# dspcraft/dsc

Measured on AMD Instinct MI355X. Metric: batched 1-D rfft GSamples/s, higher is better.
Workload: dtype f32

## Files before the change

### dsc_amd/csrc/check_store_hazard.py

```python
#!/usr/bin/env python3
import os
import re
import struct
import subprocess
import sys
import tempfile

LLVM = '/opt/rocm/lib/llvm/bin'
BUNDLE_MAGIC = b'__CLANG_OFFLOAD_BUNDLE__'

_STORE = re.compile(r'^(buffer|global|flat|scratch)_store_(dwordx3|dwordx4|b96|b128)\s+(.*)$')
_VREG = re.compile(r'v\[(\d+):(\d+)\]|v(\d+)\b')
_NOP = re.compile(r'^s_nop\s+(\d+)')


def _vrange(tok):
    m = _VREG.match(tok.strip())
    if not m:
        return None
    if m.group(3) is not None:
        return int(m.group(3)), int(m.group(3))
    return int(m.group(1)), int(m.group(2))


def _valu_dest(instr):
    if not instr.startswith('v_'):
        return None
    op, _, rest = instr.partition(' ')
    if op.startswith(('v_cmp', 'v_cmpx', 'v_readlane', 'v_readfirstlane', 'v_nop')):
        return None
    first = rest.split(',')[0]
    return _vrange(first)


def device_code_objects(path):
    data = open(path, 'rb').read()
    found = False
    pos = 0
    while True:
        i = data.find(BUNDLE_MAGIC, pos)
        if i < 0:
            break
        n = struct.unpack_from('<Q', data, i + 24)[0]
        off = i + 32
        for _ in range(n):
            o, size, tsz = struct.unpack_from('<QQQ', data, off)
            off += 24
            triple = data[off:off + tsz].decode()
            off += tsz
            if 'amdgcn' in triple and size:
                found = True
                yield f'{os.path.basename(path)}@{i + o}', data[i + o:i + o + size]
        pos = i + 24
    if not found and data[:4] == b'\x7fELF' and data[18:20] == b'\xe0\x00':
        yield os.path.basename(path), data


def disassemble(blob):
    with tempfile.NamedTemporaryFile(suffix='.co') as f:
        f.write(blob)
        f.flush()
        out = subprocess.run([f'{LLVM}/llvm-objdump', '-d', '--no-show-raw-insn', '--no-leading-addr', f.name], check=True, capture_output=True, text=True).stdout
    return out


def scan_text(asm, label=''):
    stores = 0
    bad = []
    func = '?'
    lines = []
    for raw in asm.splitlines():
        s = raw.split('//')[0].split(';')[0].strip()
        if not s:
            continue
        if s.endswith(':') and not s.startswith(('v_', 's_', 'buffer_', 'global_', 'ds_', 'flat_', 'scratch_')):
            func = s.rstrip(':').strip('<>')
            m = re.match(r'^[0-9a-f]+ <(.*)>$', func)
            if m:
                func = m.group(1)
            lines.append(('label', func))
            continue
        lines.append(('i', s))
    cur = '?'
    for idx, (kind, s) in enumerate(lines):
        if kind == 'label':
            if not s.startswith(('.L', 'L')):
                cur = s
            continue
        m = _STORE.match(s)
        if not m:
            continue
        ops = [o.strip() for o in m.group(3).split(',')]
        data = _vrange(ops[0] if m.group(1) == 'buffer' else (ops[1] if len(ops) > 1 else ''))
        if data is None:
            continue
        stores += 1
        need = 2 if m.group(1) == 'buffer' else 1
        ws = 0
        k = idx + 1
        while ws < need and k < len(lines):
            kind2, t = lines[k]
            k += 1
            if kind2 == 'label':
                continue
            d = _valu_dest(t)
            if d is not None and d[0] <= data[1] and d[1] >= data[0]:
                bad.append(f'{label} {cur}: `{s}` then, {ws} wait state(s) later, `{t}`')
                break
            nop = _NOP.match(t)
            ws += int(nop.group(1)) + 1 if nop else 1
            if t.startswith(('s_endpgm', 's_branch', 's_setpc')):
                break
    return stores, bad


def scan_file(path):
    total, bad = 0, []
    for label, blob in device_code_objects(path):
        n, b = scan_text(disassemble(blob), label)
        total += n
        bad += b
    return total, bad


def main(argv):
    total, bad = 0, []
    for p in argv:
        n, b = scan_file(p)
        total += n
        bad += b
    print(f'check_store_hazard: {total} stores of more than 64 bits, {len(bad)} with a VALU write to their data registers inside the wait states')
    for line in bad[:40]:
        print('  ' + line)
    return 1 if bad or total == 0 else 0


if __name__ == '__main__':
    sys.exit(main(sys.argv[1:]))
```

### dsc_amd/csrc/fft_c2c_32k.hip

```cpp
#define DSC_R2C64K_HELPERS_ONLY 1
#include "fft_r2c_64k.hip"

namespace {

template<bool INV, bool CAST>
__global__ __launch_bounds__(1024) void c2c32k_kernel(const f2 *__restrict__ z, f2 *__restrict__ Z, int batch, const f2 *__restrict__ aux,
                                                      int in_pitch, int in_len) {
    constexpr int EB = CAST ? 4 : 8;
    auto sample = [](__amdgpu_buffer_rsrc_t r, int voff, int soff) {
        if constexpr (CAST) return cf{__builtin_bit_cast(float, __builtin_amdgcn_raw_buffer_load_b32(r, voff, soff, kStream)), 0.0f};
        else return load_c(r, voff, soff);
    };
    extern __shared__ __attribute__((aligned(16))) float lds[];
    float *plane = lds;
    f2 *T = (f2 *) (lds + kPlaneFloats);
    fill_twiddle_table(T, aux);
    const int wave_sgpr = __builtin_amdgcn_readfirstlane(threadIdx.x >> 6);
    constexpr float kScale = 1.0f / (float) kM;

    cf v[32];
    {
        const int row0 = blockIdx.x;
        const __amdgpu_buffer_rsrc_t r0 = __builtin_amdgcn_make_buffer_rsrc(
            (void *) ((const char *) z + (size_t) row0 * in_pitch * EB), 0, row0 < batch ? in_len * EB : 0, 0x00020000);
        const int load_off = thread_id(wave_sgpr) * EB;
#pragma unroll
        for (int a = 0; a < 32; ++a) v[a] = sample(r0, load_off, a * 1024 * EB);
    }
    for (int row = blockIdx.x; row < batch; row += gridDim.x) {
        const int next_row = row + gridDim.x;
        const __amdgpu_buffer_rsrc_t rnext = __builtin_amdgcn_make_buffer_rsrc(
            (void *) ((const char *) z + (size_t) next_row * in_pitch * EB), 0, next_row < batch ? in_len * EB : 0, 0x00020000);
        const __amdgpu_buffer_rsrc_t rout = __builtin_amdgcn_make_buffer_rsrc((void *) (Z + (size_t) row * kM), 0, kM * 8, 0x00020000);
        three_passes<INV>(v, plane, T, aux, wave_sgpr, wave_sgpr, false, false);
        if (INV) {
#pragma unroll
            for (int p = 0; p < 32; ++p) v[p] = cf{v[p].x * kScale, v[p].y * kScale};
        }
        const int load_off = thread_id(wave_sgpr) * EB;
        staged_time_store(v, plane, rout, wave_sgpr, [&](bool first_half) {
            if (first_half) {
#pragma unroll
                for (int a = 0; a < 16; ++a) v[2 * a] = sample(rnext, load_off, a * 1024 * EB);
            } else {
#pragma unroll
                for (int a = 16; a < 32; ++a) v[2 * (a - 16) + 1] = sample(rnext, load_off, a * 1024 * EB);
            }
        });
        unzip_rows(v);
    }
}

}

void dsc_launch_fft32k_c32(const void *z, void *Z, int batch, int in_pitch, int in_len, bool inverse, bool cast, const void *aux, int n_cu,
                           hipStream_t stream) {
    if (batch <= 0) return;
    const int grid = batch < n_cu ? batch : n_cu;
    with_bool(inverse, [&](auto inv) { with_bool(cast, [&](auto c) {
        dsc_launch_dyn_lds<c2c32k_kernel<decltype(inv)::value, decltype(c)::value>>(grid, 1024, kLdsBytes, stream, (const f2 *) z, (f2 *) Z, batch,
                                                                                    (const f2 *) aux, in_pitch, in_len);
    }); });
}
```

### dsc_amd/csrc/fft_r2c_64k.hip

```cpp
#include "dispatch.h"

#include <hip/hip_runtime.h>

#include <cmath>
#include <cstdlib>
#include <utility>

namespace {

typedef float f2 __attribute__((ext_vector_type(2)));

struct cf { float x, y; };
__device__ __forceinline__ cf operator+(cf a, cf b) { return cf{a.x + b.x, a.y + b.y}; }
__device__ __forceinline__ cf operator-(cf a, cf b) { return cf{a.x - b.x, a.y - b.y}; }
__device__ __forceinline__ cf to_cf(f2 a) { return cf{a.x, a.y}; }
__device__ __forceinline__ f2 to_f2(cf a) { return f2{a.x, a.y}; }

constexpr int kM = 32768;
constexpr int kPlaneFloats = 1024 * 34;
constexpr int kLdsBytes = kPlaneFloats * 4 + 1024 * 8;
constexpr int kTabEntries = 1024;

constexpr int kAuxW1024 = 0, kAuxW32768 = 1024, kAuxW65536 = 2048, kAuxEntries = 3072;

__host__ __device__ constexpr int br5(int x) {
    return ((x & 1) << 4) | ((x & 2) << 2) | (x & 4) | ((x & 8) >> 2) | ((x & 16) >> 4);
}

__device__ constexpr float kCos64[17] = {
    1.0f, 0.99518472667219688624f, 0.98078528040323044913f, 0.95694033573220886494f,
    0.92387953251128675613f, 0.88192126434835502971f, 0.83146961230254523708f, 0.77301045336273696081f,
    0.70710678118654752440f, 0.63439328416364549822f, 0.55557023301960222474f, 0.47139673682599764856f,
    0.38268343236508977173f, 0.29028467725446236764f, 0.19509032201612826785f, 0.09801714032956060199f,
    0.0f};

__device__ constexpr float root64_re(int q) {
    q &= 63;
    return q <= 16 ? kCos64[q] : q <= 32 ? -kCos64[32 - q] : q <= 48 ? -kCos64[q - 32] : kCos64[64 - q];
}
__device__ constexpr float root64_im(int q) {
    q &= 63;
    return q <= 16 ? -kCos64[16 - q] : q <= 32 ? -kCos64[q - 16] : q <= 48 ? kCos64[48 - q] : kCos64[q - 48];
}

__device__ __forceinline__ cf cmul(cf a, cf w) {
    return cf{a.x * w.x - a.y * w.y, a.x * w.y + a.y * w.x};
}
__device__ __forceinline__ cf cmul_conj(cf a, cf w) {
    return cf{a.x * w.x + a.y * w.y, a.y * w.x - a.x * w.y};
}

template<bool INV>
__device__ __forceinline__ cf twiddle_mul_second_fused(cf a, cf w) {
    if (INV) return cf{__builtin_fmaf(a.y, w.y, a.x * w.x), __builtin_fmaf(-a.x, w.y, a.y * w.x)};
    return cf{__builtin_fmaf(-a.y, w.y, a.x * w.x), __builtin_fmaf(a.y, w.x, a.x * w.y)};
}

template<bool INV, int M, int K>
__device__ __forceinline__ cf mul_root(cf d) {
    constexpr float c8 = 0.70710678118654752440f;
    if constexpr (K == 0) {
        return d;
    } else if constexpr (4 * K == M) {
        return INV ? cf{-d.y, d.x} : cf{d.y, -d.x};
    } else if constexpr (8 * K == M) {
        return INV ? cf{(d.x - d.y) * c8, (d.x + d.y) * c8} : cf{(d.x + d.y) * c8, (d.y - d.x) * c8};
    } else if constexpr (8 * K == 3 * M) {
        return INV ? cf{-(d.x + d.y) * c8, (d.x - d.y) * c8} : cf{(d.y - d.x) * c8, -(d.x + d.y) * c8};
    } else {
        constexpr float wr = root64_re(K * (64 / M));
        constexpr float wi = INV ? -root64_im(K * (64 / M)) : root64_im(K * (64 / M));
        return cf{d.x * wr - d.y * wi, d.x * wi + d.y * wr};
    }
}
// ... 118 lines not shown
#endif

typedef unsigned int u2 __attribute__((ext_vector_type(2)));
typedef unsigned int u4 __attribute__((ext_vector_type(4)));
typedef float f4 __attribute__((ext_vector_type(4)));

#ifndef DSC_LDS_SPLIT_READS
#define DSC_LDS_SPLIT_READS 1
#endif
__device__ __forceinline__ f2 lds_read_b64(const f2 *p) {
#if DSC_LDS_SPLIT_READS
    return *(const volatile __attribute__((address_space(3))) f2 *) p;
#else
    return *p;
#endif
}

__device__ __forceinline__ void lds_barrier() {
    __builtin_amdgcn_fence(__ATOMIC_RELEASE, "workgroup", "local");
    __builtin_amdgcn_s_barrier();
    __builtin_amdgcn_fence(__ATOMIC_ACQUIRE, "workgroup", "local");
}

__device__ __forceinline__ float bperm(int byte_addr, float x) {
    return __int_as_float(__builtin_amdgcn_ds_bpermute(byte_addr, __float_as_int(x)));
}

__device__ __forceinline__ int column_of(int wave, int lane) {
    int kp = lane < 32 ? 32 * wave + lane : 1024 - 32 * wave - (63 - lane);
    return kp == 1024 ? 512 : kp;
}

#ifdef DSC_R2C64K_PROBE
#define PROBE_ARGS , int io_on
#define PROBE_NULL , 1
#define IO_ON io_on
#else
#define PROBE_ARGS
#define PROBE_NULL
#define IO_ON 1
#endif

__device__ __forceinline__ int thread_id(int wave_sgpr) {
    int zero;
    asm volatile("v_mov_b32 %0, 0" : "=v"(zero));
    const int lane = __builtin_amdgcn_mbcnt_hi(-1, __builtin_amdgcn_mbcnt_lo(-1, zero));
    return (wave_sgpr << 6) | lane;
}

#ifndef DSC_STREAM_AUX
#define DSC_STREAM_AUX 2
#endif
constexpr int kStream = DSC_STREAM_AUX;
__device__ __forceinline__ cf load_c(__amdgpu_buffer_rsrc_t r, int voff, int soff) {
    return to_cf(__builtin_bit_cast(f2, __builtin_amdgcn_raw_buffer_load_b64(r, voff, soff, kStream)));
}
#ifndef DSC_FILTER_EARLY_LOADS
#define DSC_FILTER_EARLY_LOADS 4
#endif
#ifndef DSC_IRFFT_PIN_PASS3
#define DSC_IRFFT_PIN_PASS3 1
#endif
#ifndef DSC_IRFFT_EARLY_PAIRS
#define DSC_IRFFT_EARLY_PAIRS 4
#endif
#ifndef DSC_IRFFT_LOAD_AUX
#define DSC_IRFFT_LOAD_AUX 0
#endif
__device__ __forceinline__ cf load_c_spec(__amdgpu_buffer_rsrc_t r, int voff, int soff) {
    return to_cf(__builtin_bit_cast(f2, __builtin_amdgcn_raw_buffer_load_b64(r, voff, soff, DSC_IRFFT_LOAD_AUX)));
}
__device__ __forceinline__ cf load_c_cached(__amdgpu_buffer_rsrc_t r, int voff, int soff) {
    return to_cf(__builtin_bit_cast(f2, __builtin_amdgcn_raw_buffer_load_b64(r, voff, soff, 0)));
}
template<int POLICY>
__device__ __forceinline__ void store_c(cf a, __amdgpu_buffer_rsrc_t r, int voff, int soff) {
    __builtin_amdgcn_raw_buffer_store_b64(__builtin_bit_cast(u2, to_f2(a)), r, voff, soff, POLICY);
}

__device__ __forceinline__ void fill_twiddle_table(f2 *T, const f2 *aux) {
    const int t = threadIdx.x;
    T[t] = aux[kAuxW1024 + (t >> 5) * (t & 31)];
    __syncthreads();
}

constexpr int kCPitch = 33;
static_assert(512 * kCPitch * 8 <= kPlaneFloats * 4, "the step buffer lives inside the plane");

__host__ __device__ constexpr int class_of(int k) { return (k ^ (k >> 1)) & 1; }
__host__ __device__ constexpr int index_in_class(int k) { return ((k >> 2) << 1) | (k & 1); }
static_assert(class_of(br5(0)) == 0 && class_of(br5(7)) == 0 && class_of(br5(24)) == 0 && class_of(br5(31)) == 0 &&
              class_of(br5(8)) == 1 && class_of(br5(23)) == 1, "class 0 = quarters 0 and 3 of a dft32 output");

__device__ __forceinline__ int reader_column(int t) {
    const int a = t >> 5;
    return (t & 31) | ((((a >> 3) | ((a & 7) << 2))) << 5);
}
__device__ __forceinline__ int spectrum_wave(int wave_sgpr) { return (wave_sgpr >> 2) | ((wave_sgpr & 3) << 2); }

template<int Q>
__device__ __forceinline__ void quarter_write(f2 *buf, int wbase, const cf (&v)[32]) {
    int wbase_hi = wbase + 8 * (32 * kCPitch);
    asm("" : "+v"(wbase_hi));
    f2 *lo8 = buf + wbase;
    f2 *hi8 = buf + wbase_hi;
#pragma unroll
    for (int p = 8 * Q; p < 8 * Q + 8; ++p)
        if (index_in_class(br5(p)) < 8) lo8[index_in_class(br5(p)) * (32 * kCPitch)] = to_f2(v[p]);
#pragma unroll
    for (int p = 8 * Q; p < 8 * Q + 8; ++p)
        if (index_in_class(br5(p)) >= 8) hi8[(index_in_class(br5(p)) - 8) * (32 * kCPitch)] = to_f2(v[p]);
}

__device__ __forceinline__ void step_read(const f2 *buf, int row, cf (&dst)[32]) {
    const f2 *r = buf + __mul24(row, kCPitch);
#pragma unroll
    for (int m = 0; m < 32; ++m) dst[m] = to_cf(lds_read_b64(r + m));
}

__device__ __forceinline__ void pin(cf (&v)[32]) {
#pragma unroll
    for (int p = 0; p < 32; p += 8)
        asm volatile("" : "+v"(v[p].x), "+v"(v[p].y), "+v"(v[p + 1].x), "+v"(v[p + 1].y), "+v"(v[p + 2].x), "+v"(v[p + 2].y), "+v"(v[p + 3].x),
                     "+v"(v[p + 3].y), "+v"(v[p + 4].x), "+v"(v[p + 4].y), "+v"(v[p + 5].x), "+v"(v[p + 5].y), "+v"(v[p + 6].x), "+v"(v[p + 6].y),
                     "+v"(v[p + 7].x), "+v"(v[p + 7].y));
}

template<typename Finish>
__device__ __forceinline__ void exchange(f2 *buf, int wbase, int rclass, int rrow, cf (&src)[32], cf (&dst)[32], Finish finish) {
    pin(src);
    lds_barrier();
    finish(std::integral_constant<int, 0>{});
    quarter_write<0>(buf, wbase, src);
    finish(std::integral_constant<int, 3>{});
    quarter_write<3>(buf, wbase, src);
    lds_barrier();
    cf r[32];
    if (rclass == 0) step_read(buf, rrow, r);
    finish(std::integral_constant<int, 1>{});
    lds_barrier();
    quarter_write<1>(buf, wbase, src);
    finish(std::integral_constant<int, 2>{});
    quarter_write<2>(buf, wbase, src);
    lds_barrier();
    if (rclass != 0) step_read(buf, rrow, r);
#pragma unroll
    for (int m = 0; m < 32; ++m) dst[m] = r[m];
}

struct no_hook { __device__ __forceinline__ void operator()() const {} };

template<bool INV, typename Hook = no_hook>
__device__ __forceinline__ void three_passes(cf (&v)[32], float *plane, const f2 *T, const f2 *aux, int wave_sgpr, int col_wave,
                                             bool mirrored_in, bool mirrored_out, Hook before_pass3 = Hook{}) {
    f2 *buf = (f2 *) plane;
    const int wave_class = ((wave_sgpr >> 2) ^ (wave_sgpr >> 3)) & 1;
    dft32_head<INV>(v);
    cf u[32];
    {
        const int t = thread_id(wave_sgpr);
        const int col = mirrored_in ? column_of(col_wave, t & 63) : t;
        const int hi = col >> 5;
        const f2 *th = T + hi;
        const int rc = reader_column(t);
        exchange(buf, __mul24(col & 31, kCPitch) + hi, wave_class, (index_in_class(rc >> 5) << 5) | (rc & 31), v, u, [&](auto Q) {
            constexpr int kQ = decltype(Q)::value;
            dft32_quarter<INV, kQ>(v);
#pragma unroll
            for (int p = 8 * kQ; p < 8 * kQ + 8; ++p) {
                if (p == 0) continue;
                const cf w = to_cf(th[32 * br5(p)]);
                v[p] = INV ? cmul_conj(v[p], w) : cmul(v[p], w);
            }
        });
    }
    dft32_head<INV>(u);
    {
        const int t = thread_id(wave_sgpr);
        const int rc = reader_column(t);
        const int hi = rc >> 5, lo = rc & 31;
        const cf tw2_base = to_cf(aux[kAuxW32768 + __mul24(hi, lo)]);
        const f2 *tl = T + lo;
        const int col_out = mirrored_out ? column_of(col_wave, t & 63) : rc;
        const int k2 = col_out >> 5;
        const int rclass = mirrored_out ? class_of(k2) : wave_class;
        exchange(buf, __mul24(hi, kCPitch) + lo, rclass, (index_in_class(k2) << 5) | (col_out & 31), u, v, [&](auto Q) {
            constexpr int kQ = decltype(Q)::value;
            dft32_quarter<INV, kQ>(u);
#ifdef DSC_DFT32_DIF
            constexpr bool kSumsOnly = false;
#else
            constexpr bool kSumsOnly = true;
#endif
#pragma unroll
            for (int p = 8 * kQ; p < 8 * kQ + 8; ++p) {
                const cf w = p == 0 ? tw2_base : cmul(tw2_base, to_cf(tl[32 * br5(p)]));
                if (kSumsOnly && p < 4) u[p] = twiddle_mul_second_fused<INV>(u[p], w);
                else u[p] = INV ? cmul_conj(u[p], w) : cmul(u[p], w);
            }
        });
    }
    before_pass3();
    dft32<INV>(v);
}

__device__ __forceinline__ void real_pair(cf p, cf q, cf wq, float hs, cf &out_k, cf &out_mk) {
    const cf s = cf{p.x + q.x, p.y - q.y};
    const cf d = cf{p.x - q.x, p.y + q.y};
    const cf wd = cmul(d, wq);
    out_k = cf{hs * s.x + wd.x, hs * s.y + wd.y};
    out_mk = cf{hs * s.x - wd.x, wd.y - hs * s.y};
}

__device__ __forceinline__ int partner_byte_addr(int wave, int lane) {
    return ((wave == 0 && (lane == 63 || lane == 0)) ? lane : 63 - lane) * 4;
}

#ifndef DSC_R2C64K_HELPERS_ONLY
__global__ __launch_bounds__(1024) void rfft64k_kernel(const float *__restrict__ x, f2 *__restrict__ X, int batch,
                                                       const f2 *__restrict__ aux, int in_pitch, int in_len PROBE_ARGS) {
    extern __shared__ __attribute__((aligned(16))) float lds[];
    float *plane = lds;
    f2 *T = (f2 *) (lds + kPlaneFloats);
    fill_twiddle_table(T, aux);

    const int wave_sgpr = __builtin_amdgcn_readfirstlane(threadIdx.x >> 6);

    cf v[32];
    {
        const int row0 = blockIdx.x;
        const __amdgpu_buffer_rsrc_t r0 = __builtin_amdgcn_make_buffer_rsrc(
            (void *) (x + (size_t) row0 * in_pitch), 0, row0 < batch ? in_len * 4 * IO_ON : 0, 0x00020000);
        const int load_off = thread_id(wave_sgpr) * 8;
#pragma unroll
        for (int j1 = 0; j1 < 32; ++j1) v[j1] = load_c(r0, load_off, j1 * 8192);
    }

    for (int row = blockIdx.x; row < batch; row += gridDim.x) {
        const int next_row = row + gridDim.x;
        const __amdgpu_buffer_rsrc_t rnext = __builtin_amdgcn_make_buffer_rsrc(
            (void *) (x + (size_t) next_row * in_pitch), 0, next_row < batch ? in_len * 4 * IO_ON : 0, 0x00020000);
        const __amdgpu_buffer_rsrc_t rout =
            __builtin_amdgcn_make_buffer_rsrc((void *) (X + (size_t) row * (kM + 1)), 0, (kM + 1) * 8 * IO_ON, 0x00020000);

        const int cw = spectrum_wave(wave_sgpr);
        three_passes<false>(v, plane, T, aux, wave_sgpr, cw, false, true);

        const int t4 = thread_id(wave_sgpr);
        const int lane = t4 & 63, wave = t4 >> 6;
        const int kp = column_of(cw, lane);
        const int partner_addr = partner_byte_addr(cw, lane);
        cf xk[16], xm[16];
        const cf zmid = v[br5(16)];
        if (cw == 0) {
#pragma unroll
            for (int r = 16; r < 31; ++r) v[br5(r)] = lane == 0 ? v[br5(r + 1)] : v[br5(r)];
            v[br5(31)] = lane == 0 ? v[br5(0)] : v[br5(31)];
        }
#pragma unroll
        for (int k3 = 0; k3 < 16; ++k3) {
            const int src = 31 - br5(k3);
            xm[k3].x = bperm(partner_addr, v[src].x);
            xm[k3].y = bperm(partner_addr, v[src].y);
        }
        {
            const cf wpost = to_cf(aux[kAuxW65536 + kp]);
            const cf post_base = cf{0.5f * wpost.y, -0.5f * wpost.x};
#pragma unroll
            for (int k3 = 0; k3 < 16; ++k3) {
                const cf c = cf{root64_re(k3), root64_im(k3)};
                const cf w = k3 == 0 ? post_base : cmul(post_base, c);
                real_pair(v[br5(k3)], xm[k3], w, 0.5f, xk[k3], xm[k3]);
            }
        }

        f2 *stage = (f2 *) plane;
        const int skew = (int) ((((size_t) (X + (size_t) row * (kM + 1))) >> 3) & 15);
        lds_barrier();
#pragma unroll
        for (int k3 = 0; k3 < 16; ++k3) stage[kp + 1024 * k3] = to_f2(xk[k3]);
        const cf xk15 = xk[15];
        const int load_off = thread_id(wave_sgpr) * 8;
#pragma unroll
        for (int j1 = 0; j1 < 16; ++j1) v[j1] = load_c(rnext, load_off, j1 * 8192);
        lds_barrier();
#pragma unroll
        for (int m = 0; m < 8; ++m) {
            const int k = 2 * (t4 + 1024 * m) - skew;
            if (m > 0 || k >= 0) {
                const f2 lo2 = lds_read_b64(stage + k), hi2 = lds_read_b64(stage + k + 1);
                const f4 q = f4{lo2.x, lo2.y, hi2.x, hi2.y};
                __builtin_amdgcn_raw_buffer_store_b128(__builtin_bit_cast(u4, q), rout, k * 8, 0, kStream);
            } else if (m == 0 && k == -1) {
                __builtin_amdgcn_raw_buffer_store_b64(__builtin_bit_cast(u2, stage[0]), rout, 0, 0, kStream);
            }
            if (m & 1) __builtin_amdgcn_sched_barrier(0);
        }
        lds_barrier();
        constexpr int kStage2 = kM / 2 - 16;
#pragma unroll
        for (int k3 = 0; k3 < 16; ++k3) stage[(kM - kStage2) - kp - 1024 * k3] = to_f2(xm[k3]);
        if (kp >= 1009) stage[kp + 15 * 1024 - kStage2] = to_f2(xk15);
        if (t4 == 0) stage[kM / 2 - kStage2] = f2{zmid.x, -zmid.y};
#pragma unroll
        for (int j1 = 16; j1 < 32; ++j1) v[j1] = load_c(rnext, load_off, j1 * 8192);
        lds_barrier();
#pragma unroll
        for (int m = 0; m < 9; ++m) {
            if (m == 8 && wave != 0) break;
            const int k = kM / 2 + 2 * (t4 + 1024 * m) - skew;
            if (m < 8 || k + 1 <= kM) {
                const f2 lo2 = lds_read_b64(stage + k - kStage2), hi2 = lds_read_b64(stage + k + 1 - kStage2);
                const f4 q = f4{lo2.x, lo2.y, hi2.x, hi2.y};
                __builtin_amdgcn_raw_buffer_store_b128(__builtin_bit_cast(u4, q), rout, k * 8, 0, kStream);
            } else if (m == 8 && k == kM) {
                __builtin_amdgcn_raw_buffer_store_b64(__builtin_bit_cast(u2, stage[k - kStage2]), rout, k * 8, 0, kStream);
            }
            if (m & 1) __builtin_amdgcn_sched_barrier(0);
        }
    }
}

#endif

__device__ __forceinline__ void inverse_prepass_direct(cf (&v)[32], cf y_mid, const f2 *aux, int wave_sgpr) {
    constexpr float kScale = 1.0f / (float) kM;
    const int t1 = thread_id(wave_sgpr);
    const int lane = t1 & 63, wave = t1 >> 6;
    const int c = column_of(wave, lane);
    const int partner_addr = partner_byte_addr(wave, lane);
    if (wave == 0 && lane == 0) { v[0].y = 0.f; v[16].y = 0.f; }
    const cf wpre = to_cf(aux[kAuxW65536 + c]);
    const cf wq_base = cf{0.5f * kScale * wpre.y, 0.5f * kScale * wpre.x};
#pragma unroll
    for (int half = 0; half < 2; ++half) {
        cf zm[8];
#pragma unroll
        for (int i = 0; i < 8; ++i) {
            const int a = half * 8 + i;
            const cf cj = cf{root64_re(a), -root64_im(a)};
            const cf wq = a == 0 ? wq_base : cmul(wq_base, cj);
            real_pair(v[a], v[16 + a], wq, 0.5f * kScale, v[a], zm[i]);
        }
#pragma unroll
        for (int i = 0; i < 8; ++i) {
            const int a = half * 8 + i;
            v[16 + a].x = bperm(partner_addr, zm[i].x);
            v[16 + a].y = bperm(partner_addr, zm[i].y);
        }
    }
    cf w[32];
#pragma unroll
    for (int r = 0; r < 16; ++r) { w[r] = v[r]; w[16 + r] = v[31 - r]; }
    if (wave == 0) {
#pragma unroll
        for (int r = 31; r > 16; --r) w[r] = lane == 0 ? w[r - 1] : w[r];
        w[16] = lane == 0 ? cf{kScale * y_mid.x, -kScale * y_mid.y} : w[16];
    }
#pragma unroll
    for (int r = 0; r < 32; ++r) v[r] = w[r];
}

template<typename IssueNext>
__device__ __forceinline__ void staged_time_store(cf (&v)[32], float *plane, __amdgpu_buffer_rsrc_t rout, int wave_sgpr,
                                                  IssueNext issue_next) {
    f2 *stage = (f2 *) plane;
    const int t4 = thread_id(wave_sgpr);
    const int c4 = reader_column(t4);
    lds_barrier();
#pragma unroll
    for (int p = 0; p < 32; p += 2) stage[c4 + 1024 * br5(p)] = to_f2(v[p]);
    issue_next(true);
    lds_barrier();
#pragma unroll
    for (int m = 0; m < 8; ++m) {
        const int k = 2 * (t4 + 1024 * m);
        const f2 lo2 = lds_read_b64(stage + k), hi2 = lds_read_b64(stage + k + 1);
        const f4 q = f4{lo2.x, lo2.y, hi2.x, hi2.y};
        __builtin_amdgcn_raw_buffer_store_b128(__builtin_bit_cast(u4, q), rout, k * 8, 0, kStream);
        if (m & 1) __builtin_amdgcn_sched_barrier(0);
    }
    lds_barrier();
#pragma unroll
    for (int p = 1; p < 32; p += 2) stage[c4 + 1024 * (br5(p) - 16)] = to_f2(v[p]);
    issue_next(false);
    lds_barrier();
#pragma unroll
    for (int m = 0; m < 8; ++m) {
        const int k = 2 * (t4 + 1024 * m);
        const f2 lo2 = lds_read_b64(stage + k), hi2 = lds_read_b64(stage + k + 1);
        const f4 q = f4{lo2.x, lo2.y, hi2.x, hi2.y};
        __builtin_amdgcn_raw_buffer_store_b128(__builtin_bit_cast(u4, q), rout, (kM / 2 + k) * 8, 0, kStream);
        if (m & 1) __builtin_amdgcn_sched_barrier(0);
    }
}

__device__ __forceinline__ void unzip_rows(cf (&v)[32]) {
    cf nxt[32];
#pragma unroll
    for (int a = 0; a < 16; ++a) { nxt[a] = v[2 * a]; nxt[16 + a] = v[2 * a + 1]; }
#pragma unroll
    for (int a = 0; a < 32; ++a) v[a] = nxt[a];
}

#ifndef DSC_R2C64K_HELPERS_ONLY
__global__ __launch_bounds__(1024) void irfft64k_kernel(const f2 *__restrict__ X, float *__restrict__ x, int batch,
                                                        const f2 *__restrict__ aux, int in_pitch, int in_len PROBE_ARGS) {
    extern __shared__ __attribute__((aligned(16))) float lds[];
    float *plane = lds;
    f2 *T = (f2 *) (lds + kPlaneFloats);
    fill_twiddle_table(T, aux);

    const int wave_sgpr = __builtin_amdgcn_readfirstlane(threadIdx.x >> 6);

    cf v[32];
    cf y_mid = cf{0.f, 0.f};
    {
        const int row0 = blockIdx.x;
        const __amdgpu_buffer_rsrc_t r0 = __builtin_amdgcn_make_buffer_rsrc(
            (void *) (X + (size_t) row0 * in_pitch), 0, row0 < batch ? in_len * 8 * IO_ON : 0, 0x00020000);
        const int t0 = thread_id(wave_sgpr);
        const int c = column_of(t0 >> 6, t0 & 63);
        const int pv = (kM - c - 15 * 1024) * 8;
#pragma unroll
        for (int a = 0; a < 16; ++a) {
            v[a] = load_c_spec(r0, c * 8, a * 8192);
            v[16 + a] = load_c_spec(r0, pv, (15 - a) * 8192);
        }
        if (c == 0) y_mid = load_c_spec(r0, (kM / 2) * 8, 0);
    }

    for (int row = blockIdx.x; row < batch; row += gridDim.x) {
        const int next_row = row + gridDim.x;
        const __amdgpu_buffer_rsrc_t rnext = __builtin_amdgcn_make_buffer_rsrc(
            (void *) (X + (size_t) next_row * in_pitch), 0, next_row < batch ? in_len * 8 * IO_ON : 0, 0x00020000);
        const __amdgpu_buffer_rsrc_t rout =
            __builtin_amdgcn_make_buffer_rsrc((void *) (x + (size_t) row * 65536), 0, 65536 * 4 * IO_ON, 0x00020000);

        inverse_prepass_direct(v, y_mid, aux, wave_sgpr);
        constexpr int kEarly = DSC_IRFFT_EARLY_PAIRS;
        cf early[kEarly > 0 ? 2 * kEarly : 1];
        three_passes<true>(v, plane, T, aux, wave_sgpr, wave_sgpr, true, false, [&]() {
            if constexpr (kEarly > 0) {
                const int t3 = thread_id(wave_sgpr);
                const int c3 = column_of(t3 >> 6, t3 & 63);
                const int pv3 = (kM - c3 - 15 * 1024) * 8;
#pragma unroll
                for (int a = 0; a < kEarly; ++a) {
                    early[2 * a] = load_c_spec(rnext, c3 * 8, a * 8192);
                    early[2 * a + 1] = load_c_spec(rnext, pv3, (15 - a) * 8192);
                }
            }
        });

#if DSC_IRFFT_PIN_PASS3
#pragma unroll
        for (int p = 0; p < 32; p += 8)
            asm volatile("" : "+v"(v[p].x), "+v"(v[p].y), "+v"(v[p + 1].x), "+v"(v[p + 1].y), "+v"(v[p + 2].x), "+v"(v[p + 2].y), "+v"(v[p + 3].x),
                         "+v"(v[p + 3].y), "+v"(v[p + 4].x), "+v"(v[p + 4].y), "+v"(v[p + 5].x), "+v"(v[p + 5].y), "+v"(v[p + 6].x), "+v"(v[p + 6].y),
                         "+v"(v[p + 7].x), "+v"(v[p + 7].y));
#endif
        const int t4 = thread_id(wave_sgpr);
        const int c = column_of(t4 >> 6, t4 & 63);
        const int pv = (kM - c - 15 * 1024) * 8;
        staged_time_store(v, plane, rout, wave_sgpr, [&](bool first_half) {
            if (first_half) {
                y_mid = cf{0.f, 0.f};
                if (c == 0) y_mid = load_c_spec(rnext, (kM / 2) * 8, 0);
#pragma unroll
                for (int i = 0; i < 8; ++i) {
                    v[2 * i] = load_c_spec(rnext, c * 8, (kEarly + i) * 8192);
                    v[16 + 2 * i] = load_c_spec(rnext, pv, (15 - kEarly - i) * 8192);
                }
            } else {
#pragma unroll
                for (int i = 0; i < 8 - kEarly; ++i) {
                    v[2 * i + 1] = load_c_spec(rnext, c * 8, (kEarly + 8 + i) * 8192);
                    v[17 + 2 * i] = load_c_spec(rnext, pv, (7 - kEarly - i) * 8192);
                }
            }
        });
        {
            cf nxt[32];
#pragma unroll
            for (int a = 0; a < 16; ++a) {
                if (a < kEarly)          { nxt[a] = early[2 * a];             nxt[16 + a] = early[2 * a + 1]; }
                else if (a < kEarly + 8) { nxt[a] = v[2 * (a - kEarly)];      nxt[16 + a] = v[16 + 2 * (a - kEarly)]; }
                else                     { nxt[a] = v[2 * (a - kEarly - 8) + 1]; nxt[16 + a] = v[17 + 2 * (a - kEarly - 8)]; }
            }
#pragma unroll
            for (int a = 0; a < 32; ++a) v[a] = nxt[a];
        }
    }
}

__global__ __launch_bounds__(1024) void filter64k_kernel(const float *__restrict__ x, const f2 *__restrict__ H,
                                                         float *__restrict__ y, int batch, const f2 *__restrict__ aux, int in_pitch,
                                                         int in_len) {
    extern __shared__ __attribute__((aligned(16))) float lds[];
    float *plane = lds;
    f2 *T = (f2 *) (lds + kPlaneFloats);
    fill_twiddle_table(T, aux);

    const int wave_sgpr = __builtin_amdgcn_readfirstlane(threadIdx.x >> 6);
    const __amdgpu_buffer_rsrc_t rh = __builtin_amdgcn_make_buffer_rsrc((void *) H, 0, (kM + 1) * 8, 0x00020000);
    constexpr float kScale = 1.0f / (float) kM;

    cf v[32];
    {
        const int row0 = blockIdx.x;
        const __amdgpu_buffer_rsrc_t r0 = __builtin_amdgcn_make_buffer_rsrc(
            (void *) (x + (size_t) row0 * in_pitch), 0, row0 < batch ? in_len * 4 : 0, 0x00020000);
        const int load_off = thread_id(wave_sgpr) * 8;
#pragma unroll
        for (int j1 = 0; j1 < 32; ++j1) v[j1] = load_c(r0, load_off, j1 * 8192);
    }
    for (int row = blockIdx.x; row < batch; row += gridDim.x) {
        const int next_row = row + gridDim.x;
        const __amdgpu_buffer_rsrc_t rnext = __builtin_amdgcn_make_buffer_rsrc(
            (void *) (x + (size_t) next_row * in_pitch), 0, next_row < batch ? in_len * 4 : 0, 0x00020000);
        const __amdgpu_buffer_rsrc_t rout =
            __builtin_amdgcn_make_buffer_rsrc((void *) (y + (size_t) row * 65536), 0, 65536 * 4, 0x00020000);
        const int cw = spectrum_wave(wave_sgpr);
        three_passes<false>(v, plane, T, aux, wave_sgpr, cw, false, true);

        {
            const int t1 = thread_id(wave_sgpr);
            const int lane = t1 & 63, wave = cw;
            const int c = column_of(wave, lane);
            const int partner_addr = partner_byte_addr(wave, lane);
            const cf wc = to_cf(aux[kAuxW65536 + c]);
            const cf post_base = cf{0.5f * wc.y, -0.5f * wc.x};
            const cf pre_base = cf{0.5f * kScale * wc.y, 0.5f * kScale * wc.x};
            if (wave == 0) {
                const cf zmid = v[br5(16)];
                const cf hmid = load_c_cached(rh, (kM / 2) * 8, 0);
                const cf pmid = cmul(cf{zmid.x, -zmid.y}, hmid);
                v[br5(16)] = lane == 0 ? cf{kScale * pmid.x, -kScale * pmid.y} : v[br5(16)];
            }
            cf park = v[br5(16)];
            if (wave == 0) {
#pragma unroll
                for (int r = 16; r < 31; ++r) v[br5(r)] = lane == 0 ? v[br5(r + 1)] : v[br5(r)];
                v[br5(31)] = lane == 0 ? v[br5(0)] : v[br5(31)];
            }
#pragma unroll
            for (int part = 0; part < 8; ++part) {
                cf q[2], zm[2];
#pragma unroll
                for (int i = 0; i < 2; ++i) {
                    const int a = part * 2 + i;
                    q[i].x = bperm(partner_addr, v[br5(31 - a)].x);
                    q[i].y = bperm(partner_addr, v[br5(31 - a)].y);
                }
#pragma unroll
                for (int i = 0; i < 2; ++i) {
                    const int a = part * 2 + i;
                    const cf w64 = cf{root64_re(a), root64_im(a)};
                    cf xk, xm;
                    real_pair(v[br5(a)], q[i], a == 0 ? post_base : cmul(post_base, w64), 0.5f, xk, xm);
                    const cf hk = load_c_cached(rh, c * 8, a * 8192);
                    const cf hm = load_c_cached(rh, (kM - 15 * 1024 - c) * 8, (15 - a) * 8192);
                    cf pk = cmul(xk, hk), pm = cmul(xm, hm);
                    if (a == 0) {
                        pk.y = (c == 0) ? 0.f : pk.y;
                        pm.y = (c == 0) ? 0.f : pm.y;
                    }
                    const cf w64c = cf{root64_re(a), -root64_im(a)};
                    real_pair(pk, pm, a == 0 ? pre_base : cmul(pre_base, w64c), 0.5f * kScale, v[br5(a)], zm[i]);
                }
#pragma unroll
                for (int i = 0; i < 2; ++i) {
                    const int a = part * 2 + i;
                    v[br5(31 - a)].x = bperm(partner_addr, zm[i].x);
                    v[br5(31 - a)].y = bperm(partner_addr, zm[i].y);
                }
                __builtin_amdgcn_sched_barrier(0);
            }
            if (wave == 0) {
#pragma unroll
                for (int r = 31; r > 16; --r) v[br5(r)] = lane == 0 ? v[br5(r - 1)] : v[br5(r)];
                v[br5(16)] = lane == 0 ? park : v[br5(16)];
            }
        }
        cf z[32];
#pragma unroll
        for (int r = 0; r < 32; ++r) z[r] = v[br5(r)];
        constexpr int kEarlyX = DSC_FILTER_EARLY_LOADS;
        cf early[kEarlyX > 0 ? kEarlyX : 1];
        three_passes<true>(z, plane, T, aux, wave_sgpr, cw, true, false, [&]() {
            if constexpr (kEarlyX > 0) {
                const int off = thread_id(wave_sgpr) * 8;
#pragma unroll
                for (int j1 = 0; j1 < kEarlyX; ++j1) early[j1] = load_c(rnext, off, j1 * 8192);
            }
        });
        {
            const int load_off = thread_id(wave_sgpr) * 8;
            staged_time_store(z, plane, rout, wave_sgpr, [&](bool first_half) {
                if (first_half) {
#pragma unroll
                    for (int i = 0; i < 16; ++i) z[2 * i] = load_c(rnext, load_off, (kEarlyX + i) * 8192);
                } else {
#pragma unroll
                    for (int i = 0; i < 16 - kEarlyX; ++i) z[2 * i + 1] = load_c(rnext, load_off, (kEarlyX + 16 + i) * 8192);
                }
            });
#pragma unroll
            for (int j1 = 0; j1 < 32; ++j1) v[j1] = j1 < kEarlyX ? early[j1] : j1 < kEarlyX + 16 ? z[2 * (j1 - kEarlyX)] : z[2 * (j1 - kEarlyX - 16) + 1];
        }
    }
}

#endif

}

#ifndef DSC_R2C64K_HELPERS_ONLY
size_t dsc_r2c64k_table_bytes() { return (size_t) kAuxEntries * sizeof(float) * 2; }

void dsc_r2c64k_build_tables(void *host_dst) {
    float *o = (float *) host_dst;
    auto put = [&](int at, long long k, long long n) {
        const long double a = -2.0L * 3.14159265358979323846264338327950288L * (long double) k / (long double) n;
        o[2 * at] = (float) cosl(a);
        o[2 * at + 1] = (float) sinl(a);
    };
    for (int m = 0; m < kTabEntries; ++m) {
        put(kAuxW1024 + m, m, 1024);
        put(kAuxW32768 + m, m, 32768);
        put(kAuxW65536 + m, m, 65536);
    }
    o[2 * (kAuxW1024 + 256)] = 0.f;  o[2 * (kAuxW1024 + 256) + 1] = -1.f;
    o[2 * (kAuxW1024 + 512)] = -1.f; o[2 * (kAuxW1024 + 512) + 1] = 0.f;
    o[2 * (kAuxW1024 + 768)] = 0.f;  o[2 * (kAuxW1024 + 768) + 1] = 1.f;
}

void dsc_launch_rfft64k(const float *x, void *X, int batch, int in_pitch, int in_len, const void *aux, int n_cu, hipStream_t stream) {
    if (batch <= 0) return;
    const int grid = batch < n_cu ? batch : n_cu;
    dsc_launch_dyn_lds<rfft64k_kernel>(grid, 1024, kLdsBytes, stream, x, (f2 *) X, batch, (const f2 *) aux, in_pitch, in_len PROBE_NULL);
}

void dsc_launch_irfft64k(const void *X, float *x, int batch, int in_pitch, int in_len, const void *aux, int n_cu, hipStream_t stream) {
    if (batch <= 0) return;
    const int grid = batch < n_cu ? batch : n_cu;
    dsc_launch_dyn_lds<irfft64k_kernel>(grid, 1024, kLdsBytes, stream, (const f2 *) X, x, batch, (const f2 *) aux, in_pitch, in_len PROBE_NULL);
}
void dsc_launch_filter64k(const float *s, const void *H, float *y, int batch, int in_pitch, int in_len, const void *aux, int n_cu,
                          hipStream_t stream) {
    if (batch <= 0) return;
    const int grid = batch < n_cu ? batch : n_cu;
    dsc_launch_dyn_lds<filter64k_kernel>(grid, 1024, kLdsBytes, stream, s, (const f2 *) H, y, batch, (const f2 *) aux, in_pitch, in_len);
}
#endif
```

Baseline: 667.0.

## Rotate persistent row loops so loads and stores share one stage; cache twiddles in LDS

```diff
diff --git a/dsc_amd/csrc/check_store_hazard.py b/dsc_amd/csrc/check_store_hazard.py
--- a/dsc_amd/csrc/check_store_hazard.py
+++ b/dsc_amd/csrc/check_store_hazard.py
@@ -23,14 +23,23 @@
     return int(m.group(1)), int(m.group(2))
 
 
-def _valu_dest(instr):
+def _valu_dests(instr):
     if not instr.startswith('v_'):
-        return None
+        return []
     op, _, rest = instr.partition(' ')
     if op.startswith(('v_cmp', 'v_cmpx', 'v_readlane', 'v_readfirstlane', 'v_nop')):
-        return None
-    first = rest.split(',')[0]
-    return _vrange(first)
+        return []
+    ops = rest.split(',')
+    written = ops[:2] if op.startswith('v_swap') else ops[:1]
+    return [r for r in (_vrange(o) for o in written) if r is not None]
+
+
+def _valu_dest(instr):
+    d = _valu_dests(instr)
+    return d[0] if d else None
+
+
+_BRANCH = re.compile(r'^(s_branch|s_cbranch_\w+)\s+(\S+)')
 
 
 def device_code_objects(path):
@@ -60,7 +69,8 @@
     with tempfile.NamedTemporaryFile(suffix='.co') as f:
         f.write(blob)
         f.flush()
-        out = subprocess.run([f'{LLVM}/llvm-objdump', '-d', '--no-show-raw-insn', '--no-leading-addr', f.name], check=True, capture_output=True, text=True).stdout
+        out = subprocess.run([f'{LLVM}/llvm-objdump', '-d', '--no-show-raw-insn', '--no-leading-addr', '--symbolize-operands', f.name],
+                             check=True, capture_output=True, text=True).stdout
     return out
 
 
@@ -81,6 +91,7 @@
             lines.append(('label', func))
             continue
         lines.append(('i', s))
+    label_at = {s: i for i, (kind, s) in enumerate(lines) if kind == 'label'}
     cur = '?'
     for idx, (kind, s) in enumerate(lines):
         if kind == 'label':
@@ -96,21 +107,32 @@
             continue
         stores += 1
         need = 2 if m.group(1) == 'buffer' else 1
-        ws = 0
-        k = idx + 1
-        while ws < need and k < len(lines):
-            kind2, t = lines[k]
-            k += 1
-            if kind2 == 'label':
-                continue
-            d = _valu_dest(t)
-            if d is not None and d[0] <= data[1] and d[1] >= data[0]:
-                bad.append(f'{label} {cur}: `{s}` then, {ws} wait state(s) later, `{t}`')
-                break
-            nop = _NOP.match(t)
-            ws += int(nop.group(1)) + 1 if nop else 1
-            if t.startswith(('s_endpgm', 's_branch', 's_setpc')):
-                break
+        paths = [(idx + 1, 0)]
+        seen = set()
+        hit = False
+        while paths and not hit:
+            k, ws = paths.pop()
+            while ws < need and k < len(lines) and (k, ws) not in seen:
+                seen.add((k, ws))
+                kind2, t = lines[k]
+                k += 1
+                if kind2 == 'label':
+                    continue
+                if any(d[0] <= data[1] and d[1] >= data[0] for d in _valu_dests(t)):
+                    bad.append(f'{label} {cur}: `{s}` then, {ws} wait state(s) later, `{t}`')
+                    hit = True
+                    break
+                nop = _NOP.match(t)
+                ws += int(nop.group(1)) + 1 if nop else 1
+                if t.startswith(('s_endpgm', 's_setpc')):
+                    break
+                br = _BRANCH.match(t)
+                if br:
+                    target = label_at.get(br.group(2))
+                    if target is not None:
+                        paths.append((target, ws))
+                    if br.group(1) == 's_branch':
+                        break
     return stores, bad
 
 
diff --git a/dsc_amd/csrc/fft_c2c_32k.hip b/dsc_amd/csrc/fft_c2c_32k.hip
--- a/dsc_amd/csrc/fft_c2c_32k.hip
+++ b/dsc_amd/csrc/fft_c2c_32k.hip
@@ -19,24 +19,12 @@
     constexpr float kScale = 1.0f / (float) kM;
 
     cf v[32];
-    {
-        const int row0 = blockIdx.x;
-        const __amdgpu_buffer_rsrc_t r0 = __builtin_amdgcn_make_buffer_rsrc(
-            (void *) ((const char *) z + (size_t) row0 * in_pitch * EB), 0, row0 < batch ? in_len * EB : 0, 0x00020000);
-        const int load_off = thread_id(wave_sgpr) * EB;
 #pragma unroll
-        for (int a = 0; a < 32; ++a) v[a] = sample(r0, load_off, a * 1024 * EB);
-    }
-    for (int row = blockIdx.x; row < batch; row += gridDim.x) {
-        const int next_row = row + gridDim.x;
-        const __amdgpu_buffer_rsrc_t rnext = __builtin_amdgcn_make_buffer_rsrc(
-            (void *) ((const char *) z + (size_t) next_row * in_pitch * EB), 0, next_row < batch ? in_len * EB : 0, 0x00020000);
-        const __amdgpu_buffer_rsrc_t rout = __builtin_amdgcn_make_buffer_rsrc((void *) (Z + (size_t) row * kM), 0, kM * 8, 0x00020000);
-        three_passes<INV>(v, plane, T, aux, wave_sgpr, wave_sgpr, false, false);
-        if (INV) {
-#pragma unroll
-            for (int p = 0; p < 32; ++p) v[p] = cf{v[p].x * kScale, v[p].y * kScale};
-        }
+    for (int p = 0; p < 32; ++p) v[p] = cf{0.f, 0.f};
+    for (int row = blockIdx.x;; row += gridDim.x) {
+        const int prev_row = row - (int) gridDim.x;
+        const __amdgpu_buffer_rsrc_t rnext = row_rsrc(z, row, batch, (size_t) in_pitch * EB, in_len * EB);
+        const __amdgpu_buffer_rsrc_t rout = row_rsrc(Z, prev_row, batch, (size_t) kM * 8, kM * 8);
         const int load_off = thread_id(wave_sgpr) * EB;
         staged_time_store(v, plane, rout, wave_sgpr, [&](bool first_half) {
             if (first_half) {
@@ -48,6 +36,13 @@
             }
         });
         unzip_rows(v);
+        if (row >= batch) break;
+
+        three_passes<INV>(v, plane, T, wave_sgpr, wave_sgpr, false, false);
+        if (INV) {
+#pragma unroll
+            for (int p = 0; p < 32; ++p) v[p] = cf{v[p].x * kScale, v[p].y * kScale};
+        }
     }
 }
 
diff --git a/dsc_amd/csrc/fft_r2c_64k.hip b/dsc_amd/csrc/fft_r2c_64k.hip
--- a/dsc_amd/csrc/fft_r2c_64k.hip
+++ b/dsc_amd/csrc/fft_r2c_64k.hip
@@ -17,9 +17,13 @@
 __device__ __forceinline__ f2 to_f2(cf a) { return f2{a.x, a.y}; }
 
 constexpr int kM = 32768;
-constexpr int kPlaneFloats = 1024 * 34;
-constexpr int kLdsBytes = kPlaneFloats * 4 + 1024 * 8;
+constexpr int kPlaneFloats = 1024 * 33;
 constexpr int kTabEntries = 1024;
+constexpr int kLdsW32768 = kTabEntries, kLdsW65536 = 2 * kTabEntries;
+constexpr int kLdsParked = 3 * kTabEntries;
+constexpr int kLdsBytes = kPlaneFloats * 4 + (3 * kTabEntries + 1) * 8;
+static_assert(kLdsBytes <= 160 * 1024, "one workgroup per CU: all of its LDS");
+static_assert((kM / 2 + 17) * 8 <= kPlaneFloats * 4, "the store staging area (half a spectrum row and its 17 extra bins) lives inside the plane");
 
 constexpr int kAuxW1024 = 0, kAuxW32768 = 1024, kAuxW65536 = 2048, kAuxEntries = 3072;
 
@@ -244,6 +248,12 @@
 #define DSC_STREAM_AUX 2
 #endif
 constexpr int kStream = DSC_STREAM_AUX;
+
+__device__ __forceinline__ __amdgpu_buffer_rsrc_t row_rsrc(const void *base, int row, int batch, size_t pitch_bytes, int valid_bytes) {
+    const bool in_batch = (unsigned) row < (unsigned) batch;
+    return __builtin_amdgcn_make_buffer_rsrc((void *) ((size_t) base + (size_t) ((long long) row * (long long) pitch_bytes)), 0,
+                                             in_batch ? valid_bytes : 0, 0x00020000);
+}
 __device__ __forceinline__ cf load_c(__amdgpu_buffer_rsrc_t r, int voff, int soff) {
     return to_cf(__builtin_bit_cast(f2, __builtin_amdgcn_raw_buffer_load_b64(r, voff, soff, kStream)));
 }
@@ -273,6 +283,8 @@
 __device__ __forceinline__ void fill_twiddle_table(f2 *T, const f2 *aux) {
     const int t = threadIdx.x;
     T[t] = aux[kAuxW1024 + (t >> 5) * (t & 31)];
+    T[kLdsW32768 + t] = aux[kAuxW32768 + t];
+    T[kLdsW65536 + t] = aux[kAuxW65536 + t];
     __syncthreads();
 }
 
@@ -284,10 +296,19 @@
 static_assert(class_of(br5(0)) == 0 && class_of(br5(7)) == 0 && class_of(br5(24)) == 0 && class_of(br5(31)) == 0 &&
               class_of(br5(8)) == 1 && class_of(br5(23)) == 1, "class 0 = quarters 0 and 3 of a dft32 output");
 
-__device__ __forceinline__ int reader_column(int t) {
+__host__ __device__ constexpr int reader_column(int t) {
     const int a = t >> 5;
     return (t & 31) | ((((a >> 3) | ((a & 7) << 2))) << 5);
 }
+__host__ __device__ constexpr int reader_column(int wave, int lane) {
+    return (((wave >> 2) | ((wave & 3) << 3)) << 5) | (lane & 31) | ((lane & 32) << 2);
+}
+constexpr bool reader_column_forms_agree() {
+    for (int t = 0; t < 1024; ++t)
+        if (reader_column(t) != reader_column(t >> 6, t & 63)) return false;
+    return true;
+}
+static_assert(reader_column_forms_agree(), "reader_column(wave, lane) == reader_column(64 wave + lane)");
 __device__ __forceinline__ int spectrum_wave(int wave_sgpr) { return (wave_sgpr >> 2) | ((wave_sgpr & 3) << 2); }
 
 template<int Q>
@@ -340,11 +361,9 @@
     for (int m = 0; m < 32; ++m) dst[m] = r[m];
 }
 
-struct no_hook { __device__ __forceinline__ void operator()() const {} };
-
-template<bool INV, typename Hook = no_hook>
-__device__ __forceinline__ void three_passes(cf (&v)[32], float *plane, const f2 *T, const f2 *aux, int wave_sgpr, int col_wave,
-                                             bool mirrored_in, bool mirrored_out, Hook before_pass3 = Hook{}) {
+template<bool INV>
+__device__ __forceinline__ void first_two_passes(cf (&v)[32], float *plane, const f2 *T, int wave_sgpr, int col_wave, bool mirrored_in,
+                                                 bool mirrored_out) {
     f2 *buf = (f2 *) plane;
     const int wave_class = ((wave_sgpr >> 2) ^ (wave_sgpr >> 3)) & 1;
     dft32_head<INV>(v);
@@ -371,7 +390,7 @@
         const int t = thread_id(wave_sgpr);
         const int rc = reader_column(t);
         const int hi = rc >> 5, lo = rc & 31;
-        const cf tw2_base = to_cf(aux[kAuxW32768 + __mul24(hi, lo)]);
+        const cf tw2_base = to_cf(T[kLdsW32768 + __mul24(hi, lo)]);
         const f2 *tl = T + lo;
         const int col_out = mirrored_out ? column_of(col_wave, t & 63) : rc;
         const int k2 = col_out >> 5;
@@ -392,7 +411,12 @@
             }
         });
     }
-    before_pass3();
+}
+
+template<bool INV>
+__device__ __forceinline__ void three_passes(cf (&v)[32], float *plane, const f2 *T, int wave_sgpr, int col_wave, bool mirrored_in,
+                                             bool mirrored_out) {
+    first_two_passes<INV>(v, plane, T, wave_sgpr, col_wave, mirrored_in, mirrored_out);
     dft32<INV>(v);
 }
 
@@ -419,60 +443,27 @@
     const int wave_sgpr = __builtin_amdgcn_readfirstlane(threadIdx.x >> 6);
 
     cf v[32];
-    {
-        const int row0 = blockIdx.x;
-        const __amdgpu_buffer_rsrc_t r0 = __builtin_amdgcn_make_buffer_rsrc(
-            (void *) (x + (size_t) row0 * in_pitch), 0, row0 < batch ? in_len * 4 * IO_ON : 0, 0x00020000);
-        const int load_off = thread_id(wave_sgpr) * 8;
-#pragma unroll
-        for (int j1 = 0; j1 < 32; ++j1) v[j1] = load_c(r0, load_off, j1 * 8192);
-    }
-
-    for (int row = blockIdx.x; row < batch; row += gridDim.x) {
-        const int next_row = row + gridDim.x;
-        const __amdgpu_buffer_rsrc_t rnext = __builtin_amdgcn_make_buffer_rsrc(
-            (void *) (x + (size_t) next_row * in_pitch), 0, next_row < batch ? in_len * 4 * IO_ON : 0, 0x00020000);
-        const __amdgpu_buffer_rsrc_t rout =
-            __builtin_amdgcn_make_buffer_rsrc((void *) (X + (size_t) row * (kM + 1)), 0, (kM + 1) * 8 * IO_ON, 0x00020000);
-
-        const int cw = spectrum_wave(wave_sgpr);
-        three_passes<false>(v, plane, T, aux, wave_sgpr, cw, false, true);
-
+    cf xk[16], xm[16];
+#pragma unroll
+    for (int k3 = 0; k3 < 16; ++k3) xk[k3] = xm[k3] = cf{0.f, 0.f};
+    const int cw = spectrum_wave(wave_sgpr);
+
+    for (int row = blockIdx.x;; row += gridDim.x) {
+        const int prev_row = row - (int) gridDim.x;
+        const __amdgpu_buffer_rsrc_t rnext = row_rsrc(x, row, batch, (size_t) in_pitch * 4, in_len * 4 * IO_ON);
+        const __amdgpu_buffer_rsrc_t rout = row_rsrc(X, prev_row, batch, (size_t) (kM + 1) * 8, (kM + 1) * 8 * IO_ON);
+        {
         const int t4 = thread_id(wave_sgpr);
-        const int lane = t4 & 63, wave = t4 >> 6;
-        const int kp = column_of(cw, lane);
-        const int partner_addr = partner_byte_addr(cw, lane);
-        cf xk[16], xm[16];
-        const cf zmid = v[br5(16)];
-        if (cw == 0) {
-#pragma unroll
-            for (int r = 16; r < 31; ++r) v[br5(r)] = lane == 0 ? v[br5(r + 1)] : v[br5(r)];
-            v[br5(31)] = lane == 0 ? v[br5(0)] : v[br5(31)];
-        }
-#pragma unroll
-        for (int k3 = 0; k3 < 16; ++k3) {
-            const int src = 31 - br5(k3);
-            xm[k3].x = bperm(partner_addr, v[src].x);
-            xm[k3].y = bperm(partner_addr, v[src].y);
-        }
-        {
-            const cf wpost = to_cf(aux[kAuxW65536 + kp]);
-            const cf post_base = cf{0.5f * wpost.y, -0.5f * wpost.x};
-#pragma unroll
-            for (int k3 = 0; k3 < 16; ++k3) {
-                const cf c = cf{root64_re(k3), root64_im(k3)};
-                const cf w = k3 == 0 ? post_base : cmul(post_base, c);
-                real_pair(v[br5(k3)], xm[k3], w, 0.5f, xk[k3], xm[k3]);
-            }
-        }
-
+        const int wave = t4 >> 6;
+        const int kp = column_of(cw, t4 & 63);
         f2 *stage = (f2 *) plane;
-        const int skew = (int) ((((size_t) (X + (size_t) row * (kM + 1))) >> 3) & 15);
+        const int skew = (int) ((((size_t) X + (size_t) ((long long) prev_row * ((kM + 1) * 8))) >> 3) & 15);
         lds_barrier();
 #pragma unroll
         for (int k3 = 0; k3 < 16; ++k3) stage[kp + 1024 * k3] = to_f2(xk[k3]);
         const cf xk15 = xk[15];
-        const int load_off = thread_id(wave_sgpr) * 8;
+        const int load_off = t4 * 8;
+        __builtin_amdgcn_sched_barrier(0);
 #pragma unroll
         for (int j1 = 0; j1 < 16; ++j1) v[j1] = load_c(rnext, load_off, j1 * 8192);
         lds_barrier();
@@ -493,7 +484,11 @@
 #pragma unroll
         for (int k3 = 0; k3 < 16; ++k3) stage[(kM - kStage2) - kp - 1024 * k3] = to_f2(xm[k3]);
         if (kp >= 1009) stage[kp + 15 * 1024 - kStage2] = to_f2(xk15);
-        if (t4 == 0) stage[kM / 2 - kStage2] = f2{zmid.x, -zmid.y};
+        if (t4 == 0) {
+            const f2 zmid = T[kLdsParked];
+            stage[kM / 2 - kStage2] = f2{zmid.x, -zmid.y};
+        }
+        __builtin_amdgcn_sched_barrier(0);
 #pragma unroll
         for (int j1 = 16; j1 < 32; ++j1) v[j1] = load_c(rnext, load_off, j1 * 8192);
         lds_barrier();
@@ -510,19 +505,51 @@
             }
             if (m & 1) __builtin_amdgcn_sched_barrier(0);
         }
-    }
-}
-
-#endif
-
-__device__ __forceinline__ void inverse_prepass_direct(cf (&v)[32], cf y_mid, const f2 *aux, int wave_sgpr) {
+        }
+        if (row >= batch) break;
+
+        three_passes<false>(v, plane, T, wave_sgpr, cw, false, true);
+
+        asm volatile("" : "+v"(v[0].x));
+        const int t5 = thread_id(wave_sgpr);
+        const int lane = t5 & 63;
+        const int kp = column_of(cw, lane);
+        const int partner_addr = partner_byte_addr(cw, lane);
+        if (t5 == 0) T[kLdsParked] = to_f2(v[br5(16)]);
+        if (cw == 0) {
+#pragma unroll
+            for (int r = 16; r < 31; ++r) v[br5(r)] = lane == 0 ? v[br5(r + 1)] : v[br5(r)];
+            v[br5(31)] = lane == 0 ? v[br5(0)] : v[br5(31)];
+        }
+#pragma unroll
+        for (int k3 = 0; k3 < 16; ++k3) {
+            const int src = 31 - br5(k3);
+            xm[k3].x = bperm(partner_addr, v[src].x);
+            xm[k3].y = bperm(partner_addr, v[src].y);
+        }
+        {
+            const cf wpost = to_cf(T[kLdsW65536 + kp]);
+            const cf post_base = cf{0.5f * wpost.y, -0.5f * wpost.x};
+#pragma unroll
+            for (int k3 = 0; k3 < 16; ++k3) {
+                const cf c = cf{root64_re(k3), root64_im(k3)};
+                const cf w = k3 == 0 ? post_base : cmul(post_base, c);
+                real_pair(v[br5(k3)], xm[k3], w, 0.5f, xk[k3], xm[k3]);
+            }
+        }
+    }
+}
+
+#endif
+
+__device__ __forceinline__ void inverse_prepass_direct(cf (&v)[32], cf y_mid, const f2 *T, int wave_sgpr) {
     constexpr float kScale = 1.0f / (float) kM;
     const int t1 = thread_id(wave_sgpr);
     const int lane = t1 & 63, wave = t1 >> 6;
     const int c = column_of(wave, lane);
     const int partner_addr = partner_byte_addr(wave, lane);
     if (wave == 0 && lane == 0) { v[0].y = 0.f; v[16].y = 0.f; }
-    const cf wpre = to_cf(aux[kAuxW65536 + c]);
+    const cf wpre = to_cf(T[kLdsW65536 + c]);
     const cf wq_base = cf{0.5f * kScale * wpre.y, 0.5f * kScale * wpre.x};
 #pragma unroll
     for (int half = 0; half < 2; ++half) {
@@ -558,10 +585,11 @@
                                                   IssueNext issue_next) {
     f2 *stage = (f2 *) plane;
     const int t4 = thread_id(wave_sgpr);
-    const int c4 = reader_column(t4);
+    const int c4 = reader_column(wave_sgpr, t4 & 63);
     lds_barrier();
 #pragma unroll
     for (int p = 0; p < 32; p += 2) stage[c4 + 1024 * br5(p)] = to_f2(v[p]);
+    __builtin_amdgcn_sched_barrier(0);
     issue_next(true);
     lds_barrier();
 #pragma unroll
@@ -575,6 +603,7 @@
     lds_barrier();
 #pragma unroll
     for (int p = 1; p < 32; p += 2) stage[c4 + 1024 * (br5(p) - 16)] = to_f2(v[p]);
+    __builtin_amdgcn_sched_barrier(0);
     issue_next(false);
     lds_barrier();
 #pragma unroll
@@ -629,21 +658,21 @@
         const __amdgpu_buffer_rsrc_t rout =
             __builtin_amdgcn_make_buffer_rsrc((void *) (x + (size_t) row * 65536), 0, 65536 * 4 * IO_ON, 0x00020000);
 
-        inverse_prepass_direct(v, y_mid, aux, wave_sgpr);
+        inverse_prepass_direct(v, y_mid, T, wave_sgpr);
         constexpr int kEarly = DSC_IRFFT_EARLY_PAIRS;
         cf early[kEarly > 0 ? 2 * kEarly : 1];
-        three_passes<true>(v, plane, T, aux, wave_sgpr, wave_sgpr, true, false, [&]() {
-            if constexpr (kEarly > 0) {
-                const int t3 = thread_id(wave_sgpr);
-                const int c3 = column_of(t3 >> 6, t3 & 63);
-                const int pv3 = (kM - c3 - 15 * 1024) * 8;
-#pragma unroll
-                for (int a = 0; a < kEarly; ++a) {
-                    early[2 * a] = load_c_spec(rnext, c3 * 8, a * 8192);
-                    early[2 * a + 1] = load_c_spec(rnext, pv3, (15 - a) * 8192);
-                }
-            }
-        });
+        first_two_passes<true>(v, plane, T, wave_sgpr, wave_sgpr, true, false);
+        if constexpr (kEarly > 0) {
+            const int t3 = thread_id(wave_sgpr);
+            const int c3 = column_of(t3 >> 6, t3 & 63);
+            const int pv3 = (kM - c3 - 15 * 1024) * 8;
+#pragma unroll
+            for (int a = 0; a < kEarly; ++a) {
+                early[2 * a] = load_c_spec(rnext, c3 * 8, a * 8192);
+                early[2 * a + 1] = load_c_spec(rnext, pv3, (15 - a) * 8192);
+            }
+        }
+        dft32<true>(v);
 
 #if DSC_IRFFT_PIN_PASS3
 #pragma unroll
@@ -699,29 +728,46 @@
     constexpr float kScale = 1.0f / (float) kM;
 
     cf v[32];
-    {
-        const int row0 = blockIdx.x;
-        const __amdgpu_buffer_rsrc_t r0 = __builtin_amdgcn_make_buffer_rsrc(
-            (void *) (x + (size_t) row0 * in_pitch), 0, row0 < batch ? in_len * 4 : 0, 0x00020000);
-        const int load_off = thread_id(wave_sgpr) * 8;
-#pragma unroll
-        for (int j1 = 0; j1 < 32; ++j1) v[j1] = load_c(r0, load_off, j1 * 8192);
-    }
-    for (int row = blockIdx.x; row < batch; row += gridDim.x) {
-        const int next_row = row + gridDim.x;
-        const __amdgpu_buffer_rsrc_t rnext = __builtin_amdgcn_make_buffer_rsrc(
-            (void *) (x + (size_t) next_row * in_pitch), 0, next_row < batch ? in_len * 4 : 0, 0x00020000);
-        const __amdgpu_buffer_rsrc_t rout =
-            __builtin_amdgcn_make_buffer_rsrc((void *) (y + (size_t) row * 65536), 0, 65536 * 4, 0x00020000);
-        const int cw = spectrum_wave(wave_sgpr);
-        three_passes<false>(v, plane, T, aux, wave_sgpr, cw, false, true);
+    cf z[32];
+#pragma unroll
+    for (int p = 0; p < 32; ++p) z[p] = cf{0.f, 0.f};
+    const int cw = spectrum_wave(wave_sgpr);
+    for (int row = blockIdx.x;; row += gridDim.x) {
+        const int prev_row = row - (int) gridDim.x;
+        const __amdgpu_buffer_rsrc_t rnext = row_rsrc(x, row, batch, (size_t) in_pitch * 4, in_len * 4);
+        const __amdgpu_buffer_rsrc_t rout = row_rsrc(y, prev_row, batch, (size_t) 65536 * 4, 65536 * 4);
+        constexpr int kEarlyX = DSC_FILTER_EARLY_LOADS;
+        cf early[kEarlyX > 0 ? kEarlyX : 1];
+        if constexpr (kEarlyX > 0) {
+            const int off = thread_id(wave_sgpr) * 8;
+#pragma unroll
+            for (int j1 = 0; j1 < kEarlyX; ++j1) early[j1] = load_c(rnext, off, j1 * 8192);
+        }
+        dft32<true>(z);
+        {
+            const int load_off = thread_id(wave_sgpr) * 8;
+            staged_time_store(z, plane, rout, wave_sgpr, [&](bool first_half) {
+                if (first_half) {
+#pragma unroll
+                    for (int i = 0; i < 16; ++i) z[2 * i] = load_c(rnext, load_off, (kEarlyX + i) * 8192);
+                } else {
+#pragma unroll
+                    for (int i = 0; i < 16 - kEarlyX; ++i) z[2 * i + 1] = load_c(rnext, load_off, (kEarlyX + 16 + i) * 8192);
+                }
+            });
+#pragma unroll
+            for (int j1 = 0; j1 < 32; ++j1) v[j1] = j1 < kEarlyX ? early[j1] : j1 < kEarlyX + 16 ? z[2 * (j1 - kEarlyX)] : z[2 * (j1 - kEarlyX - 16) + 1];
+        }
+        if (row >= batch) break;
+
+        three_passes<false>(v, plane, T, wave_sgpr, cw, false, true);
 
         {
             const int t1 = thread_id(wave_sgpr);
             const int lane = t1 & 63, wave = cw;
             const int c = column_of(wave, lane);
             const int partner_addr = partner_byte_addr(wave, lane);
-            const cf wc = to_cf(aux[kAuxW65536 + c]);
+            const cf wc = to_cf(T[kLdsW65536 + c]);
             const cf post_base = cf{0.5f * wc.y, -0.5f * wc.x};
             const cf pre_base = cf{0.5f * kScale * wc.y, 0.5f * kScale * wc.x};
             if (wave == 0) {
@@ -775,32 +821,9 @@
                 v[br5(16)] = lane == 0 ? park : v[br5(16)];
             }
         }
-        cf z[32];
 #pragma unroll
         for (int r = 0; r < 32; ++r) z[r] = v[br5(r)];
-        constexpr int kEarlyX = DSC_FILTER_EARLY_LOADS;
-        cf early[kEarlyX > 0 ? kEarlyX : 1];
-        three_passes<true>(z, plane, T, aux, wave_sgpr, cw, true, false, [&]() {
-            if constexpr (kEarlyX > 0) {
-                const int off = thread_id(wave_sgpr) * 8;
-#pragma unroll
-                for (int j1 = 0; j1 < kEarlyX; ++j1) early[j1] = load_c(rnext, off, j1 * 8192);
-            }
-        });
-        {
-            const int load_off = thread_id(wave_sgpr) * 8;
-            staged_time_store(z, plane, rout, wave_sgpr, [&](bool first_half) {
-                if (first_half) {
-#pragma unroll
-                    for (int i = 0; i < 16; ++i) z[2 * i] = load_c(rnext, load_off, (kEarlyX + i) * 8192);
-                } else {
-#pragma unroll
-                    for (int i = 0; i < 16 - kEarlyX; ++i) z[2 * i + 1] = load_c(rnext, load_off, (kEarlyX + 16 + i) * 8192);
-                }
-            });
-#pragma unroll
-            for (int j1 = 0; j1 < 32; ++j1) v[j1] = j1 < kEarlyX ? early[j1] : j1 < kEarlyX + 16 ? z[2 * (j1 - kEarlyX)] : z[2 * (j1 - kEarlyX - 16) + 1];
-        }
+        first_two_passes<true>(z, plane, T, wave_sgpr, cw, true, false);
     }
 }
 
```

After: 667.0, median of 2. About the same (-0.0%).
